# aous72/OpenJPH

Hardware: AMD Instinct MI355X
Metric: Msamples/s encode+decode, 8K 12-bit 4:4:4; achieved HBM GB/s vs roofline (higher is better)
Workload: dtype f32; 1 GPU; c3_8k_444_12b_irv97; width=7680, height=4320, components=3, bit_depth=12, wavelet=9/7 irreversible, decomps=5, hip_streams=1, sample_container_bits=16, roundtrip_max_abs_err=8

## Files before the change

openjph_amd/csrc/kernels_ht_dec.hip:

```cpp
#include <hip/hip_runtime.h>
#include <algorithm>
#include <cstdlib>
#include <stdint.h>
#include <type_traits>
#include "../../include/ojphgpu.h"
#include "ht_quant.h"
#include "ht_tables.h"
#include "ht_uvlc.h"

namespace ojphgpu {
__device__ uint16_t g_dec_vlc[2][1024];
__device__ uint32_t g_dec_vlc32[2][1024];
__device__ uint16_t g_dec_uvlc0[320];
}

namespace {

using ojphgpu::dequantise;

constexpr int WAVES = 4;
constexpr uint32_t RING_WORDS = 256;
constexpr uint32_t RING_MASK = RING_WORDS - 1;
constexpr uint32_t RING_ALLOC = RING_WORDS + 2;
constexpr uint32_t ROW_BITS_MAX = 64 * 2 * 32;
// ... 174 lines not shown
  __device__ __forceinline__ void prefetch() { pre = w[idx < last ? idx : last]; }
  __device__ __forceinline__ void settle() {}
};

typedef __attribute__((address_space(3))) uint32_t lds_u32;
constexpr uint32_t LDS_WAIT_SPINS = 1u << 23;
constexpr uint32_t EV_WORDS = 44;
constexpr uint32_t EV_RING = 8;
__device__ __forceinline__ uint32_t ev_words_of(uint32_t QW, uint32_t QH)
{
  const uint32_t w = (QW * QH + ((QW + 1u) >> 1) + 31u) / 32u + 2u;
  return w < EV_WORDS ? w : EV_WORDS;
}

constexpr uint32_t EV_AHEAD = 4;
__device__ __forceinline__ void mel_run(uint64_t& win, uint32_t& n, uint32_t& k, uint64_t& ev, uint32_t& nev)
{
  const uint32_t e = mel_exp(k);
  const uint32_t top = (uint32_t)(win >> 32);
  const bool zr = (top >> 31) != 0u;
  const uint32_t run = (top >> (31u - e)) & ((1u << e) - 1u);
  const uint32_t adv = zr ? 1u : e + 1u;
  ev |= zr ? 0ull : 1ull << (nev + run);
  nev += zr ? 1u << e : run + 1u;
  k = zr ? (k < 12u ? k + 1u : 12u) : (k > 0u ? k - 1u : 0u);
  win <<= adv; n -= adv;
}

__device__ __forceinline__ void mel_producer(const uint32_t* __restrict__ w, uint32_t nwords, uint32_t out_words,
                                             lds_u32* s_ev, volatile lds_u32* s_prog, const volatile lds_u32* s_cons,
                                             const volatile lds_u32* s_done, uint32_t lane)
{
  const uint32_t last = nwords - 1u;
  uint64_t win = ((uint64_t)w[0] << 32) | (uint64_t)w[last < 1u ? last : 1u];
  uint32_t n = 64, idx = 2, k = 0, nev = 0, wr = 0;
  uint32_t pre = w[last < 2u ? last : 2u];
  uint64_t ev = 0;
  while (wr < out_words && s_done[lane] == 0u) {
    const bool go = wr < s_cons[lane] + EV_AHEAD;
    if (go) {
      if (n <= 32u) { win |= (uint64_t)pre << (32u - n); n += 32u; ++idx; pre = w[idx < last ? idx : last]; }
      while (nev <= 31u && n >= 6u) mel_run(win, n, k, ev, nev);
      if (nev >= 32u) {
        s_ev[(wr & (EV_RING - 1u)) * 64u + lane] = (uint32_t)ev; ev >>= 32; nev -= 32u; ++wr;
        __builtin_amdgcn_fence(__ATOMIC_RELEASE, "workgroup", "local");
        s_prog[lane] = wr;
      }
    }
    if (__ballot(go) == 0ull) __builtin_amdgcn_s_sleep(16);
  }
}

struct EvRd {
  const lds_u32* ev; volatile lds_u32* prog; volatile lds_u32* cons; uint32_t idx, last, lo, hi, pre, bp, avail, lane; bool stuck;
  __device__ __forceinline__ uint32_t fetch(uint32_t want) {
    if (want >= avail && !stuck) {
      uint32_t spins = 0;
      do { __builtin_amdgcn_s_sleep(2); avail = prog[lane]; } while (want >= avail && ++spins < LDS_WAIT_SPINS);
      __builtin_amdgcn_fence(__ATOMIC_ACQUIRE, "workgroup", "local");
      stuck = stuck || want >= avail;
    }
    return ev[(want & (EV_RING - 1u)) * 64u + lane];
  }
  __device__ __forceinline__ void init(const lds_u32* e, volatile lds_u32* p, volatile lds_u32* c, uint32_t nwords, uint32_t l) {
    ev = e; prog = p; cons = c; last = nwords - 1u; lane = l; avail = 0; stuck = false;
    lo = fetch(0); hi = fetch(last < 1u ? last : 1u); pre = fetch(last < 2u ? last : 2u);
    idx = 2; bp = 0;
  }
  __device__ __forceinline__ uint32_t peek() const { return __builtin_amdgcn_alignbit(hi, lo, bp); }
  __device__ __forceinline__ void advance(uint32_t k) {
    bp += k;
    const bool cross = bp >= 32u;
    lo = cross ? hi : lo; hi = cross ? pre : hi;
    bp = cross ? bp - 32u : bp; idx += cross ? 1u : 0u;
  }
  __device__ __forceinline__ void prefetch() { cons[lane] = idx; pre = fetch(idx < last ? idx : last); }
};

struct __attribute__((aligned(4))) U2 { uint32_t x, y; };
__device__ __forceinline__ void store_pair(uint32_t* p, uint32_t a, uint32_t b)
{
  U2 v; v.x = a; v.y = b;
  *reinterpret_cast<U2*>(p) = v;
}

constexpr uint32_t REC_STRIDE = 128;

#define PIN_WINDOW(r) asm volatile("" : "+v"((r).lo), "+v"((r).hi))

#ifndef S2_ROWS_N
#define S2_ROWS_N 8
#endif
constexpr uint32_t S2_ROWS = S2_ROWS_N, S2_MAX_PER_WAVE = 8;
struct SliceSched {
  uint32_t tail, b1, b2, max_qh, n;
  uint32_t h1, h2;
  __host__ __device__ explicit SliceSched(uint32_t mq) {
    max_qh = mq ? mq : 1u;
    tail = ((max_qh - 1u) / S2_ROWS) * S2_ROWS;
#ifndef S2_TAIL
#define S2_TAIL 2
#endif
    b1 = (S2_TAIL >= 1 && max_qh > tail + 4u) ? max_qh - 4u : tail;
    b2 = (S2_TAIL >= 2 && max_qh > b1 + 2u) ? max_qh - 2u : b1;
#ifndef S2_HEAD
#define S2_HEAD 0
#endif
    const bool head = S2_HEAD != 0 && tail >= S2_ROWS && S2_ROWS == 8u;
    h1 = !head ? 0u : S2_HEAD == 1 ? 4u : 2u;
    h2 = !head ? 0u : S2_HEAD == 2 ? 4u : 0u;
    n = tail / S2_ROWS + 1u + (b1 > tail ? 1u : 0u) + (b2 > b1 ? 1u : 0u) + (h1 ? 1u : 0u) + (h2 ? 1u : 0u);
  }
  __host__ __device__ void bounds(uint32_t sl, uint32_t& lo, uint32_t& hi) const {
    const uint32_t extra = (h1 ? 1u : 0u) + (h2 ? 1u : 0u);
    if (sl <= extra) {
      const uint32_t first_end = tail >= S2_ROWS ? S2_ROWS : 0u;
      if (extra && first_end) {
        const uint32_t c0 = 0u, c1 = h1, c2 = h2 ? h2 : first_end, c3 = first_end;
        if (sl == 0u) { lo = c0; hi = c1; return; }
        if (sl == 1u) { lo = c1; hi = c2; return; }
        lo = c2; hi = c3; return;
      }
    }
    sl -= extra;
    const uint32_t full = tail / S2_ROWS;
    if (sl < full) { lo = sl * S2_ROWS; hi = lo + S2_ROWS; return; }
    uint32_t j = sl - full;
    lo = tail;
    if (b1 > tail) { if (j == 0u) { hi = b1; return; } --j; lo = b1; }
    if (b2 > b1) { if (j == 0u) { hi = b2; return; } --j; lo = b2; }
// ... 11 lines not shown
  u32x4 q[4];
#pragma unroll
  for (uint32_t j = 0; j < 4; ++j) {
    q[j].x = s_rec[(4 * j + 0) * 64 + lane]; q[j].y = s_rec[(4 * j + 1) * 64 + lane];
    q[j].z = s_rec[(4 * j + 2) * 64 + lane]; q[j].w = s_rec[(4 * j + 3) * 64 + lane];
  }
  asm volatile("global_store_dwordx4 %0, %1, off sc1\n\tglobal_store_dwordx4 %0, %2, off offset:1024 sc1\n\t"
               "global_store_dwordx4 %0, %3, off offset:2048 sc1\n\tglobal_store_dwordx4 %0, %4, off offset:3072 sc1"
               :: "v"(dst), "v"(q[0]), "v"(q[1]), "v"(q[2]), "v"(q[3]) : "memory");
}
#ifdef FUSED_TIMELINE
__device__ uint32_t g_tl_pub[1024 * 8];
__device__ uint32_t* g_tl_flags;
#endif
__device__ __forceinline__ void publish_rows(uint32_t* flag, uint32_t epoch, uint32_t rows, uint32_t lane)
{
#ifdef FUSED_TIMELINE
  const uint32_t tl_a = (uint32_t)__builtin_amdgcn_s_memrealtime();
#endif
  asm volatile("s_waitcnt vmcnt(0)" ::: "memory");
  if (lane == (uint32_t)__builtin_ctzll(__ballot(1))) {
    st_agent(flag, (epoch << 16) | rows);
#ifdef FUSED_TIMELINE
    const uint32_t k = rows == 0xFFFFu ? 7u : (rows & 7u) ? 8u : (rows >> 3) - 1u;
    if (k < 8u) { g_tl_pub[((flag - g_tl_flags) & 1023u) * 8u + k] = (uint32_t)__builtin_amdgcn_s_memrealtime(); if (k < 4u) g_tl_pub[((flag - g_tl_flags) & 1023u) * 8u + 4u + k] = tl_a; }
#endif
  }
}

template <class VlcRd>
__device__ __forceinline__ void uvlc_extension(VlcRd& vlc, uint32_t& used, uint32_t& u0, uint32_t& u1, uint32_t b0, uint32_t b1)
{
  const bool c0 = u0 - b0 > 32u, c1 = u1 - b1 > 32u;
  if (__ballot(c0 | c1) == 0ull) return;
  vlc.settle(); vlc.advance(used); vlc.prefetch(); vlc.settle(); used = 0;
  uint32_t v = vlc.peek();
  if (c0) { u0 += (v & 0xFu) << 2; v >>= 4; used += 4u; }
  if (c1) { u1 += (v & 0xFu) << 2; used += 4u; }
}

template <int NARROW, bool FUSED = false, bool W64 = false, class VlcRd, class TblT>
__device__ __forceinline__ void step1_rows(VlcRd& vlc, EvRd& mel, uint32_t* __restrict__ rec, uint32_t QW, uint32_t QH,
                                           const TblT* s_vlc, const uint16_t* s_uvlc0, uint32_t* flag = nullptr, uint32_t epoch = 0,
                                           lds_u32* s_rec = nullptr, SliceSched sched = SliceSched(S2_ROWS))
{
  static_assert(!FUSED || NARROW == 1, "the fused launch's records are for blocks of at most 64 columns");
  typedef typename std::conditional<NARROW == 2, unsigned __int128, uint64_t>::type Mask;
  auto row16 = [&](uint32_t qy_) { return rec + (size_t)qy_ * (64u * REC16_ROW_WORDS); };
  Mask sig_prev = 0;
  const uint32_t PW = (QW + 1) >> 1;

  {
    uint32_t tleft = 0; Mask sig_cur = 0;
    for (uint32_t qx = 0; qx < QW; qx += 2) {
      uint32_t v = vlc.peek(), used = 0;
      const uint32_t evq = mel.peek(); uint32_t ecnt = 0;
      uint32_t c_q = ((tleft & 0x10u) << 3) | ((tleft & 0xE0u) << 2);
      uint32_t t0 = s_vlc[c_q + (v & 0x7Fu)];
      if (c_q == 0) { if (((evq >> ecnt) & 1u) == 0) t0 = 0; ecnt++; }
      v >>= (t0 & 7u); used += t0 & 7u;
      uint32_t t1 = 0;
      if (qx + 1 < QW) {
        c_q = ((t0 & 0x10u) << 3) | ((t0 & 0xE0u) << 2);
        t1 = s_vlc[c_q + (v & 0x7Fu)];
        if (c_q == 0) { if (((evq >> ecnt) & 1u) == 0) t1 = 0; ecnt++; }
        v >>= (t1 & 7u); used += t1 & 7u;
      }
      tleft = t1;
      if (NARROW) {
        const uint32_t nib = FUSED ? (((t0 >> 9) & 3u) | ((t1 >> 7) & 0xCu))
                                   : (((t0 >> 5) & 1u) | ((t0 >> 6) & 2u) | ((t1 >> 3) & 4u) | ((t1 >> 4) & 8u));
        sig_cur |= (Mask)nib << (2u * qx);
      }
      uint32_t mode = ((t0 & 0x8u) << 3) | ((t1 & 0x8u) << 4);
      if (mode == 0xC0u) { if ((evq >> ecnt) & 1u) mode += 0x40u; ecnt++; }
      uint32_t entry = s_uvlc0[mode + (v & 0x3Fu)];
      v >>= (entry & 7u); used += entry & 7u; entry >>= 3;
      uint32_t len = entry & 0xFu;
      const uint32_t tmp = v & ((1u << len) - 1u);
      used += len; entry >>= 4;
      len = entry & 7u; entry >>= 3;
      uint32_t u0 = 1u + (entry & 7u) + (tmp & ~(0xFFu << len));
      uint32_t u1 = 1u + (entry >> 3) + (tmp >> len);
      if (W64) { const uint32_t bias = mode == 0x100u ? 3u : 1u; uvlc_extension(vlc, used, u0, u1, bias, bias); }
      vlc.settle(); vlc.advance(used); PIN_WINDOW(vlc); vlc.prefetch(); mel.advance(ecnt); mel.prefetch();
      if (FUSED) s_rec[(qx >> 1) * 64u + vlc.lane] = (t0 >> 16) | (u0 << 9) | (t1 & 0xFFFF0000u) | (u1 << 25);
      else store_pair(rec + (size_t)(qx >> 1) * REC_STRIDE, (uint32_t)t0 | (u0 << 16), (uint32_t)t1 | (u1 << 16));
    }
    if (FUSED) flush_row16(s_rec, vlc.lane, row16(0));
    sig_prev = sig_cur;
  }
  const TblT* tbl = s_vlc + 1024;
  for (uint32_t qy = 1; qy < QH; ++qy) {
    uint32_t* row = rec + (size_t)qy * PW * REC_STRIDE;
    const uint32_t* above = row - (size_t)PW * REC_STRIDE;
    auto above_rec = [&](uint32_t q) { return above[(size_t)(q >> 1) * REC_STRIDE + (q & 1u)]; };
    uint32_t tleft = 0; Mask sig_cur = 0;
    const Mask sig_or = sig_prev | (sig_prev >> 1);
    uint32_t carry = ((uint32_t)sig_prev & 1u) << 7;
    for (uint32_t qx = 0; qx < QW; qx += 2) {
      uint32_t v = vlc.peek(), used = 0;
      const uint32_t evq = mel.peek(); uint32_t ecnt = 0;
      uint32_t k0, k1;
      if (NARROW) {
        const uint32_t w = (uint32_t)(sig_or >> (2u * qx));
        k0 = carry | ((w & 2u) << 8);
        k1 = (w & 0xAu) << 6;
        carry = (w & 8u) << 4;
      } else {
        const uint32_t up0 = above_rec(qx);
        const uint32_t upl = qx ? above_rec(qx - 1) : 0u;
        const uint32_t up1 = qx + 1 < QW ? above_rec(qx + 1) : 0u;
        const uint32_t up2 = qx + 2 < QW ? above_rec(qx + 2) : 0u;
        const uint32_t sg = ((upl >> 7) & 1u) | (((up0 >> 5) & 1u) << 1) | (((up0 >> 7) & 1u) << 2) | (((up1 >> 5) & 1u) << 3) |
                            (((up1 >> 7) & 1u) << 4) | (((up2 >> 5) & 1u) << 5);
        k0 = (((sg | (sg >> 1)) & 1u) << 7) | ((((sg >> 2) | (sg >> 3)) & 1u) << 9);
        k1 = ((((sg >> 2) | (sg >> 3)) & 1u) << 7) | ((((sg >> 4) | (sg >> 5)) & 1u) << 9);
      }
      const uint32_t c_q0 = FUSED ? ((tleft & 0x100u) | k0) : (((tleft & 0x40u) << 2) | ((tleft & 0x80u) << 1) | k0);
      uint32_t t0 = tbl[c_q0 + (v & 0x7Fu)];
      const bool z0 = c_q0 == 0;
      t0 = (z0 & ((evq & 1u) == 0)) ? 0u : t0;
      ecnt = z0 ? 1u : 0u;
      v >>= (t0 & 7u); used += t0 & 7u;
      const bool ex1 = qx + 1 < QW;
      const uint32_t c_q1 = FUSED ? ((t0 & 0x100u) | k1) : (((t0 & 0x40u) << 2) | ((t0 & 0x80u) << 1) | k1);
      uint32_t t1 = tbl[c_q1 + (v & 0x7Fu)];
      const bool z1 = ex1 & (c_q1 == 0);
      t1 = ((!ex1) | (z1 & (((evq >> ecnt) & 1u) == 0))) ? 0u : t1;
      ecnt += z1 ? 1u : 0u;
      v >>= (t1 & 7u); used += t1 & 7u;
      tleft = t1;
      if (NARROW) {
        const uint32_t nib = FUSED ? (((t0 >> 9) & 3u) | ((t1 >> 7) & 0xCu))
                                   : (((t0 >> 5) & 1u) | ((t0 >> 6) & 2u) | ((t1 >> 3) & 4u) | ((t1 >> 4) & 8u));
        sig_cur |= (Mask)nib << (2u * qx);
      }
      uint32_t u0, u1;
      used += ojphgpu::uvlc_pair_other_rows(v, t0 & 0x8u, t1 & 0x8u, u0, u1);
      if (W64) uvlc_extension(vlc, used, u0, u1, 0u, 0u);
      vlc.settle(); vlc.advance(used); PIN_WINDOW(vlc); vlc.prefetch(); mel.advance(ecnt); mel.prefetch();
      if (FUSED) s_rec[(qx >> 1) * 64u + vlc.lane] = (t0 >> 16) | (u0 << 9) | (t1 & 0xFFFF0000u) | (u1 << 25);
      else store_pair(row + (size_t)(qx >> 1) * REC_STRIDE, (uint32_t)t0 | (u0 << 16), (uint32_t)t1 | (u1 << 16));
    }
    if (FUSED) flush_row16(s_rec, vlc.lane, row16(qy));
    sig_prev = sig_cur;
    if (FUSED && sched.publishes_after(qy + 1u)) publish_rows(flag, epoch, qy + 1u, vlc.lane);
  }
}

constexpr uint32_t VR_WORDS = 16, VR_LOW = 6, EV_LOW = 2;
#ifndef MEL_RUNS_PER_PASS
#define MEL_RUNS_PER_PASS 16
#endif

struct RingRd {
  const lds_u32* ring; volatile lds_u32* prog; volatile lds_u32* cons; uint32_t idx, lo, hi, pre, bp, av, pidx, lane; bool stuck;
  __device__ __forceinline__ uint32_t fetch(uint32_t want) {
    if (stuck) return 0u;
    uint32_t avail = prog[lane], spins = 0;
    while (want >= avail && ++spins < LDS_WAIT_SPINS) { __builtin_amdgcn_s_sleep(2); avail = prog[lane]; }

    __builtin_amdgcn_fence(__ATOMIC_ACQUIRE, "workgroup", "local");
    stuck = stuck || want >= avail;
    return ring[(want & (VR_WORDS - 1u)) * 64u + lane];
  }
  __device__ __forceinline__ void init(const lds_u32* r, volatile lds_u32* p, volatile lds_u32* c, uint32_t l) {
    ring = r; prog = p; cons = c; lane = l; stuck = false;
    lo = fetch(0); hi = fetch(1); pre = fetch(2);
    idx = 2; bp = 0; pidx = 0; av = 1;
  }
  __device__ __forceinline__ uint32_t peek() const { return __builtin_amdgcn_alignbit(hi, lo, bp); }
  __device__ __forceinline__ void advance(uint32_t k) {
    bp += k;
    const bool cross = bp >= 32u;
    lo = cross ? hi : lo; hi = cross ? pre : hi;
    bp = cross ? bp - 32u : bp; idx += cross ? 1u : 0u;
  }
  __device__ __forceinline__ void prefetch() { cons[lane] = idx; pidx = idx; av = prog[lane]; pre = ring[(idx & (VR_WORDS - 1u)) * 64u + lane]; }
  __device__ __forceinline__ void settle() {
    if (pidx >= av) {
      pre = fetch(pidx); av = pidx + 1u;
    }
  }
};

struct __attribute__((aligned(4))) B16 { uint32_t d[4]; };
__device__ __forceinline__ B16 load_b16_unaligned(const uint8_t* p) { B16 v; __builtin_memcpy(&v, p, 16); return v; }

template <int ROLE>
__device__ __forceinline__ void raw_partner(const uint8_t* __restrict__ cb, uint32_t lcup, uint32_t scup, uint32_t room_below,
                                            const B16& v0, const B16& v1, uint32_t ev_words,
                                            lds_u32* s_ev, volatile lds_u32* s_eprog, const volatile lds_u32* s_econs,
                                            lds_u32* s_vr, volatile lds_u32* s_vprog, const volatile lds_u32* s_vcons,
                                            const volatile lds_u32* s_done, uint32_t lane)
{
  const uint32_t vreal = scup - 2u, vcount = vreal + 1u;
  const uint32_t d0 = cb[lcup - 2];
  uint64_t vacc = d0 >> 4;
  uint32_t vnb = 4u - ((((d0 >> 4) & 7u) == 7u) ? 1u : 0u);
  uint32_t vk = 0, vwr = 0, vp1 = d0 | 0xFu;
  bool vp1_short = false;
  auto vload = [&](uint32_t k) -> B16 {
    B16 z; z.d[0] = z.d[1] = z.d[2] = z.d[3] = 0u;
    if (k >= vcount) return z;
    const int off = (int)lcup - 18 - (int)k;
    if (off >= -(int)room_below) return load_b16_unaligned(cb + off);
    for (int j = 0; j < 16; ++j) {
      const int o = off + 15 - j;
      if (o >= 0) z.d[3 - (j >> 2)] |= (uint32_t)cb[o] << (24 - 8 * (j & 3));
    }
    return z;
  };
  B16 vcur = v0, vnext = v1;
  const uint32_t mcount = scup - 1u, moff = lcup - scup;
  auto mload = [&](uint32_t k) -> B16 {
    if (k < mcount) return load_b16_unaligned(cb + moff + k);
    B16 z; z.d[0] = z.d[1] = z.d[2] = z.d[3] = 0xFFFFFFFFu; return z;
  };
  uint64_t win = 0;
  uint32_t n = 0, mk = 0, mprev = 0, k = 0, nev = 0, ewr = 0;
// ... 68 lines not shown
template <int CH>
__global__ __launch_bounds__(192 * CH) void ht_dec_step1_raw_kernel(
    const ojphgpu_cb_desc* __restrict__ blocks, uint32_t n, const uint8_t* __restrict__ data,
    uint32_t* __restrict__ quads, uint8_t* __restrict__ block_status)
{
  __shared__ uint16_t s_vlc[2048];
  __shared__ uint16_t s_uvlc0[320];
  __shared__ uint32_t s_ev_all[CH][EV_RING * 64];
  __shared__ uint32_t s_vr_all[CH][VR_WORDS * 64];
  __shared__ uint32_t s_ctl_all[CH][5][64];
  for (int i = threadIdx.x; i < 2048; i += blockDim.x) s_vlc[i] = (&ojphgpu::g_dec_vlc[0][0])[i];
  for (int i = threadIdx.x; i < 320; i += blockDim.x) s_uvlc0[i] = ojphgpu::g_dec_uvlc0[i];
  for (int i = threadIdx.x; i < CH * 5 * 64; i += blockDim.x) (&s_ctl_all[0][0][0])[i] = 0;
  __syncthreads();

  const uint32_t lane = threadIdx.x & 63u;
  const uint32_t wv = (uint32_t)__builtin_amdgcn_readfirstlane((int)(threadIdx.x >> 6));
  const bool chain = wv < (uint32_t)CH;
  const uint32_t set = wv % (uint32_t)CH;
  lds_u32* s_ev = (lds_u32*)s_ev_all[set];
  lds_u32* s_vr = (lds_u32*)s_vr_all[set];
  volatile lds_u32* s_eprog = (volatile lds_u32*)s_ctl_all[set][0];
  volatile lds_u32* s_econs = (volatile lds_u32*)s_ctl_all[set][1];
  volatile lds_u32* s_vprog = (volatile lds_u32*)s_ctl_all[set][2];
  volatile lds_u32* s_vcons = (volatile lds_u32*)s_ctl_all[set][3];
  volatile lds_u32* s_done = (volatile lds_u32*)s_ctl_all[set][4];
  if (chain) __builtin_amdgcn_s_setprio(3);
  const uint32_t bi = (blockIdx.x * (uint32_t)CH + set) * 64u + lane;
  if (bi >= n) return;
  const ojphgpu_cb_desc d = blocks[bi];
  if (d.reversible & 4u) return;
  if (d.w == 0 || d.h == 0 || d.len1 == 0 || d.num_passes == 0) { if (chain) block_status[bi] = 0; return; }
  const uint8_t* cb = data + d.data_off;
  const uint32_t room = d.data_off > 0xFFFFu ? 0xFFFFu : (uint32_t)d.data_off;
  B16 v0, v1;
  v0.d[0] = v0.d[1] = v0.d[2] = v0.d[3] = 0u; v1 = v0;
  if (!chain && wv < 2u * (uint32_t)CH) {
    const int o0 = (int)d.len1 - 18, o1 = o0 - 16;
    if (o0 >= -(int)room) v0 = load_b16_unaligned(cb + o0);
    else for (int j = 0; j < 16; ++j) { const int o = o0 + 15 - j; if (o >= 0) v0.d[3 - (j >> 2)] |= (uint32_t)cb[o] << (24 - 8 * (j & 3)); }
    if (o1 >= -(int)room) v1 = load_b16_unaligned(cb + o1);
    else for (int j = 0; j < 16; ++j) { const int o = o1 + 15 - j; if (o >= 0) v1.d[3 - (j >> 2)] |= (uint32_t)cb[o] << (24 - 8 * (j & 3)); }
  }
  const uint32_t scup = check_block(d, cb);
  if (scup == 0) { if (chain) block_status[bi] = 1; return; }
  const uint32_t QW = ((uint32_t)d.w + 1) >> 1, QH = ((uint32_t)d.h + 1) >> 1;
  const uint32_t evw = ev_words_of(QW, QH);
  if (!chain) {
    if (wv < 2u * (uint32_t)CH) raw_partner<1>(cb, d.len1, scup, room, v0, v1, evw, s_ev, s_eprog, s_econs, s_vr, s_vprog, s_vcons, s_done, lane);
    else raw_partner<2>(cb, d.len1, scup, room, v0, v1, evw, s_ev, s_eprog, s_econs, s_vr, s_vprog, s_vcons, s_done, lane);
    return;
  }
  uint32_t* rec = quads + d.scratch_cap;
  RingRd vlc; vlc.init(s_vr, s_vprog, s_vcons, lane);
  EvRd mel; mel.init(s_ev, s_eprog, s_econs, evw, lane);
  if (__all(QW <= 32)) step1_rows<1>(vlc, mel, rec, QW, QH, s_vlc, s_uvlc0);
  else if (__all(QW <= 64)) step1_rows<2>(vlc, mel, rec, QW, QH, s_vlc, s_uvlc0);
  else step1_rows<0>(vlc, mel, rec, QW, QH, s_vlc, s_uvlc0);
  s_done[lane] = 1u;
  block_status[bi] = (mel.stuck || vlc.stuck) ? 1 : 0;
}

template <int CH, bool W64 = false>
__global__ __launch_bounds__(128 * CH) void ht_dec_step1_kernel(
    const ojphgpu_cb_desc* __restrict__ blocks, uint32_t n, const uint8_t* __restrict__ data,
    const uint32_t* __restrict__ aux, uint32_t* __restrict__ quads, uint8_t* __restrict__ block_status)
{
  __shared__ uint16_t s_vlc[2048];
  __shared__ uint16_t s_uvlc0[320];
  __shared__ uint32_t s_ev_all[CH][EV_RING * 64];
  __shared__ uint32_t s_prog_all[CH][64];
  __shared__ uint32_t s_done_all[CH][64];
  __shared__ uint32_t s_cons_all[CH][64];
  for (int i = threadIdx.x; i < 2048; i += blockDim.x) s_vlc[i] = (&ojphgpu::g_dec_vlc[0][0])[i];
  for (int i = threadIdx.x; i < 320; i += blockDim.x) s_uvlc0[i] = ojphgpu::g_dec_uvlc0[i];
  if (threadIdx.x < 64 * CH) { (&s_prog_all[0][0])[threadIdx.x] = 0; (&s_done_all[0][0])[threadIdx.x] = 0; (&s_cons_all[0][0])[threadIdx.x] = 0; }
  __syncthreads();

  const uint32_t lane = threadIdx.x & 63u;
  const uint32_t wv = (uint32_t)__builtin_amdgcn_readfirstlane((int)(threadIdx.x >> 6));
  const bool chain = wv < (uint32_t)CH;
  const uint32_t set = chain ? wv : wv - (uint32_t)CH;
  uint32_t* s_ev = s_ev_all[set];
  uint32_t* s_prog = s_prog_all[set];
  volatile lds_u32* s_done = (volatile lds_u32*)s_done_all[set];
  volatile lds_u32* s_cons = (volatile lds_u32*)s_cons_all[set];
  if (chain) __builtin_amdgcn_s_setprio(3);
  const uint32_t bi = (blockIdx.x * (uint32_t)CH + set) * 64u + lane;
  if (bi >= n) return;
  const ojphgpu_cb_desc d = blocks[bi];
  if (((d.reversible & 4u) != 0) != W64) return;
  if (d.w == 0 || d.h == 0 || d.len1 == 0 || d.num_passes == 0) { if (chain) block_status[bi] = 0; return; }
  const uint8_t* cb = data + d.data_off;
  const uint32_t scup = check_block(d, cb);
  if (scup == 0) { if (chain) block_status[bi] = 1; return; }
  const uint32_t QW = ((uint32_t)d.w + 1) >> 1, QH = ((uint32_t)d.h + 1) >> 1;
  const uint32_t evw = ev_words_of(QW, QH);
  if (!chain) {
    mel_producer(aux + d.reserved + vlc_words(scup), mel_words(scup), evw, (lds_u32*)s_ev, (volatile lds_u32*)s_prog, s_cons, s_done, lane);
    return;
  }
  uint32_t* rec = quads + d.scratch_cap;

  FlatRd vlc; vlc.init(aux + d.reserved, vlc_words(scup));
  EvRd mel; mel.init((const lds_u32*)s_ev, (volatile lds_u32*)s_prog, s_cons, evw, lane);

  if (__all(QW <= 32)) step1_rows<1, false, W64>(vlc, mel, rec, QW, QH, s_vlc, s_uvlc0);
  else if (__all(QW <= 64)) step1_rows<2, false, W64>(vlc, mel, rec, QW, QH, s_vlc, s_uvlc0);
  else step1_rows<0, false, W64>(vlc, mel, rec, QW, QH, s_vlc, s_uvlc0);
  s_done[lane] = 1u;
  block_status[bi] = mel.stuck ? 1 : 0;
}


#ifndef S2_ABL
#define S2_ABL 0
#endif
__device__ __forceinline__ bool needs_refinement(const ojphgpu_cb_desc& d)
{
  return d.num_passes > 1 && d.num_passes <= 3 && d.len2 > 0 && (d.missing_msbs < 29 || (d.reversible & 4u));
}

constexpr uint32_t S2_STATE_WORDS = 24;

#ifdef FUSED_TIMELINE
__device__ uint32_t g_tl[8192 * 12];
__device__ __forceinline__ uint32_t tl_now() { return (uint32_t)__builtin_amdgcn_s_memrealtime(); }
#endif
constexpr uint32_t TICKET_STRIDE = 32;
constexpr uint32_t TICKET_CU_WORDS = 8 * 256;
constexpr uint32_t TICKET_WORDS = TICKET_CU_WORDS + 2 * TICKET_STRIDE;

__device__ __forceinline__ uint32_t rec16_base(const ojphgpu_cb_desc& d, uint32_t bi)
{
  const uint32_t l = bi & 63u;
  return d.scratch_cap - 2u * l + l * 4u;
}

__device__ __forceinline__ void load_slice_records(const uint32_t* __restrict__ quads, const ojphgpu_cb_desc& d, uint32_t bi,
                                                   uint32_t qy_begin, uint32_t qy_end, int lane, uint32_t* ents)
{
  const uint32_t QH = ((uint32_t)d.h + 1u) >> 1;
  const uint16_t* r16 = reinterpret_cast<const uint16_t*>(quads + rec16_base(d, bi) + (size_t)qy_begin * (64u * REC16_ROW_WORDS) + ((uint32_t)lane >> 4) * 256u)
                        + (((uint32_t)lane >> 1) & 7u);
  constexpr uint32_t row_step = 2u * 64u * REC16_ROW_WORDS;
  const uint32_t last = (qy_end < QH ? qy_end : QH) - qy_begin - 1u;
#pragma unroll
  for (uint32_t i = 0; i < S2_ROWS; ++i)
    ents[i] = (uint32_t)__hip_atomic_load(r16 + (i < last ? i : last) * row_step, __ATOMIC_RELAXED, __HIP_MEMORY_SCOPE_AGENT);
}

template <int TX, int WD, bool SLICED, bool KEEP = false>
__device__ __forceinline__ void step2_block(const ojphgpu_cb_desc& d, uint32_t bi, const uint8_t* __restrict__ data,
                                            const uint32_t* __restrict__ quads, uint32_t* __restrict__ coef,
                                            uint8_t* __restrict__ block_status, uint32_t* ring, uint8_t* s_exp_w,
                                            int lane, uint32_t qy_begin, uint32_t qy_end, uint32_t* state, bool prepare = false)
{
  const uint32_t W = d.w, H = d.h, pitch = d.pitch;
  if (W == 0 || H == 0) return;
  uint32_t* dst = coef + d.coef_off;
  const bool rev = TX == 1 ? true : TX == 2 ? false : (d.reversible & 1u) != 0;
  const uint32_t K = d.K_max;
  const bool raw_out = TX ? false : needs_refinement(d);

// ... 52 lines not shown
  if (wide) for (uint32_t i = lane; i < 2 * EXP_BYTES / 4; i += 64) reinterpret_cast<uint32_t*>(s_exp_w)[i] = 0;
  wave_sync();

  uint32_t dst_bits = 0, src_pos = 0, mpos = 0;
  uint32_t hs[5] = { 0, 0, 0, 0, 0 }, hd[5] = { 0, 0, 0, 0, 0 };
  auto unstuff_chunk = [&]() {
    if (SLICED && !KEEP) {
#pragma unroll
      for (int i = 4; i > 0; --i) { hs[i] = hs[i - 1]; hd[i] = hd[i - 1]; }
      hs[0] = src_pos; hd[0] = dst_bits;
    }
    const uint32_t wb = (dst_bits + 31u) >> 5;
    {
      const uint32_t z0 = (wb + (uint32_t)lane) & RING_MASK;
      ring[z0] = 0;
      if (z0 < 2u) ring[z0 + RING_WORDS] = 0;
      if (lane < 2) { const uint32_t z1 = (wb + 64u + (uint32_t)lane) & RING_MASK; ring[z1] = 0; if (z1 < 2u) ring[z1 + RING_WORDS] = 0; }
    }
    wave_sync();
    const uint32_t i0 = src_pos + 4u * (uint32_t)lane;
    uint32_t val = 0, nb = 0;
    const uint32_t word = i0 < ms_len ? load_u32_unaligned(cb + i0) : 0u;
    uint32_t pw = from_prev(word);
    if (lane == 0) pw = (i0 && i0 < ms_len) ? load_u32_unaligned(cb + i0 - 4) : 0u;
    asm volatile("" :: "v"(word), "v"(pw));
    if (i0 < ms_len) {
      const uint32_t cnt = min(4u, ms_len - i0);
      const uint32_t valid = cnt == 4u ? 0xFFFFFFFFu : (1u << (8u * cnt)) - 1u;
      const uint32_t P = (word << 8) | (pw >> 24), P2 = (word << 16) | (pw >> 16);
      auto is_ff = [](uint32_t x) { return ((x & 0x7F7F7F7Fu) + 0x01010101u) & x & 0x80808080u; };
      const uint32_t S = is_ff(P) & valid;
      const uint32_t stray = (is_ff(P2) >> 7) & (P >> 7) & 0x01010101u;
      uint32_t x = ((word | stray) & valid) & ~S;
      x = (S & 0x00800000u) ? (x & 0x007FFFFFu) | ((x >> 1) & 0xFF800000u) : x;
      x = (S & 0x00008000u) ? (x & 0x00007FFFu) | ((x >> 1) & 0xFFFF8000u) : x;
      x = (S & 0x00000080u) ? (x & 0x0000007Fu) | ((x >> 1) & 0xFFFFFF80u) : x;
      val = x;
      nb = 8u * cnt - (uint32_t)__popc(S);
    }
    const uint32_t incl = wave_incl_scan(nb);
    const uint32_t pos = dst_bits + incl - nb;
    if (nb) {
      const uint32_t w = pos >> 5, sh = pos & 31;
      const uint32_t wa = w & RING_MASK, wb2 = (w + 1) & RING_MASK;
      atomicOr(&ring[wa], val << sh);
      if (wa < 2u) atomicOr(&ring[wa + RING_WORDS], val << sh);
      if (sh + nb > 32) { atomicOr(&ring[wb2], val >> (32 - sh)); if (wb2 < 2u) atomicOr(&ring[wb2 + RING_WORDS], val >> (32 - sh)); }
    }
    dst_bits += rdlane(incl, 63);
    src_pos += 256;
    wave_sync();
  };

  const uint32_t mmsbp2 = missing_msbs + 2;
  const uint32_t shift = 31 - K;
  const float delta = d.delta;
  const uint32_t half = (uint32_t)lane & 1u;
  bool bad = false;
  uint32_t e_prev = 0;
  if (KEEP && prepare) {
    while (src_pos < ms_len && dst_bits < ROW_BITS_MAX + 64u) unstuff_chunk();
    if (lane < 16) state[lane] = 0u;
    if (lane == 0) { state[16] = 0u; state[17] = src_pos; state[18] = dst_bits; state[19] = 0u; state[20] = ms_len; }
    wave_sync();
    return;
  }
  if (SLICED && (KEEP || qy_begin > 0)) {
    if (!KEEP && rdfirst(state[19]) != 0u) return;
    e_prev = (state[(uint32_t)lane >> 2] >> (8u * ((uint32_t)lane & 3u))) & 0xFFu;
    mpos = rdfirst(state[16]); src_pos = rdfirst(state[17]); dst_bits = rdfirst(state[18]);
    hs[0] = src_pos; hd[0] = dst_bits;
  }
  uint32_t ent_next = 0;
  if (!SLICED) {
    ent_next = (uint32_t)lane < W && qy_begin < qy_last ? rec_at(qy_begin, (uint32_t)lane >> 1) : 0u;
    asm volatile("" : "+v"(ent_next));
  }
  for (uint32_t qy = qy_begin; qy < qy_last && !bad; ++qy) {
    const uint8_t* vexp = s_exp_w + (qy & 1) * EXP_BYTES;
    uint8_t* vnew = s_exp_w + ((qy & 1) ^ 1) * EXP_BYTES;
    for (uint32_t c0 = 0; c0 < (WD == 1 ? 1u : W); c0 += 64) {
      while (!(S2_ABL & 16) && src_pos < ms_len && (int32_t)(dst_bits - mpos) < (int32_t)(ROW_BITS_MAX + 64u)) unstuff_chunk();
      const bool exhausted = src_pos >= ms_len;
      const uint32_t col = c0 + (uint32_t)lane;
      const bool act = col < W;
      const uint32_t qx = col >> 1;
      const uint32_t ent = SLICED ? ents[0] : ent_next;
      if (SLICED) {
#pragma unroll
        for (uint32_t i = 0; i + 1 < (SLICED ? S2_ROWS : 1u); ++i) ents[i] = ents[i + 1];
      } else {
        uint32_t nc0 = c0 + 64, nqy = qy;
        if (nc0 >= W) { nc0 = 0; nqy = qy + 1; }
        const uint32_t ncol = nc0 + (uint32_t)lane;
        ent_next = (nqy < qy_last && ncol < W) ? rec_at(nqy, ncol >> 1) : 0u;
      }
      const uint32_t inf = act ? (ent & 0xFFFFu) : 0u;
      uint32_t U_q = SLICED ? inf >> 9 : ent >> 16;
      if (qy > 0) {
        uint32_t gamma = SLICED ? inf & 0x100u : inf & 0xF0u;
        if (!SLICED) gamma &= gamma - 0x10u;
        uint32_t em;
        if (S2_ABL & 8) em = e_prev;
        else if (!wide) {
          const uint32_t e_nx = from_next(e_prev), e_pv = from_prev(e_prev);
          const uint32_t hm = max(e_prev, half ? e_nx : e_pv);
          em = max(hm, from_pair(hm));
        } else {
          const uint32_t b = 2 * qx;
          em = act ? max(max((uint32_t)vexp[b], (uint32_t)vexp[b + 1]), max((uint32_t)vexp[b + 2], (uint32_t)vexp[b + 3])) : 0u;
        }
        U_q += gamma ? max(em, 1u) : 1u;
      }
      if (__ballot(U_q > mmsbp2) != 0ull) { bad = true; break; }
      const uint32_t sel = SLICED ? inf >> (4u * half) : inf >> (2u * half);
      const uint32_t st0 = sel & 3u, st1 = (sel >> 2) & 3u;
      const bool sg0 = SLICED ? st0 != 0u : (sel & 0x10u) != 0u, sg1 = SLICED ? st1 != 0u : (sel & 0x20u) != 0u;
      const uint32_t ek0 = SLICED ? st0 >> 1 : (sel >> 12) & 1u, ek1 = SLICED ? st1 >> 1 : (sel >> 13) & 1u;
      const uint32_t eb0 = SLICED ? st0 & (st0 >> 1) : (sel >> 8) & 1u, eb1 = SLICED ? st1 & (st1 >> 1) : (sel >> 9) & 1u;
      const uint32_t m0 = sg0 ? U_q - ek0 : 0u;
      const uint32_t m1 = sg1 ? U_q - ek1 : 0u;
      const uint32_t tot = m0 + m1;
      const uint32_t incl = (S2_ABL & 2) ? tot * ((uint32_t)lane + 1u) : wave_incl_scan(tot);
      const uint32_t at = mpos + incl - tot;
      mpos += (S2_ABL & 2) ? 64u : rdlane(incl, 63);
      const uint32_t wi = at >> 5, sh = at & 31;
      const uint32_t* rw = ring + (wi & RING_MASK);
      const uint32_t w0 = (S2_ABL & 4) ? at : rw[0], w1 = (S2_ABL & 4) ? at * 3u : rw[1], w2 = (S2_ABL & 4) ? at * 5u : rw[2];
      uint64_t win = (uint64_t)__funnelshift_r(w0, w1, sh) | ((uint64_t)__funnelshift_r(w1, w2, sh) << 32);
      if (exhausted) {
        if (at >= dst_bits) win = ~0ull;
        else if (at + 64 > dst_bits) win |= ~0ull << (dst_bits - at);
      }
      uint32_t out0, out1, v1;
      {
        const uint32_t ms_val = (uint32_t)win;
        uint32_t v_n = ms_val & ((1u << m0) - 1u);
        v_n |= eb0 << m0;
        v_n |= 1u;
        const uint32_t val = ((ms_val << 31) | ((v_n + 2u) << (p - 1))) & (sg0 ? 0xFFFFFFFFu : 0u);
        out0 = raw_out ? val : dequantise(val, rev, shift, delta);
      }
      {
        const uint32_t ms_val = __builtin_amdgcn_alignbit((uint32_t)(win >> 32), (uint32_t)win, m0);
        uint32_t v_n = ms_val & ((1u << m1) - 1u);
        v_n |= eb1 << m1;
        v_n |= 1u;
        const uint32_t keep = sg1 ? 0xFFFFFFFFu : 0u;
        const uint32_t val = ((ms_val << 31) | ((v_n + 2u) << (p - 1))) & keep;
        v1 = v_n & keep;
        out1 = raw_out ? val : dequantise(val, rev, shift, delta);
      }
      const uint32_t e_new = v1 ? 31u - (uint32_t)__clz((int)v1) : 0u;
      if (!wide) e_prev = e_new;
      else if (act) vnew[col + 1] = (uint8_t)e_new;
      if (!SLICED) asm volatile("" : "+v"(ent_next));
      if (act && (!(S2_ABL & 1) || (out0 ^ out1) == 0x9E3779B9u)) {
        const uint32_t y = 2 * qy;
        char* rowp = reinterpret_cast<char*>(dst + (size_t)y * pitch);
        char* rowp1 = rowp + (size_t)pitch * 4u;
        uint32_t coff = col * 4u;
        asm volatile("" : "+v"(coff));
        *reinterpret_cast<uint32_t*>(rowp + coff) = out0;
        if (y + 1 < H) { asm volatile("" : "+v"(coff)); *reinterpret_cast<uint32_t*>(rowp1 + coff) = out1; }
      }
    }
    if (wide) wave_sync();
  }
  if (bad) { zero_block(); if (lane == 0) block_status[bi] = 1; }
  if (SLICED && qy_last < QH) {
    if (bad) { if (lane == 0) state[19] = 1u; wave_sync(); return; }
    uint32_t rs = hs[4], rd = hd[4];
#pragma unroll
    for (int i = 3; i >= 0; --i) if (hd[i] <= mpos) { rs = hs[i]; rd = hd[i]; }
    if (KEEP) { rs = src_pos; rd = dst_bits; }
    const uint32_t e4 = e_prev | (from_next(e_prev) << 8);
    const uint32_t e8 = e4 | ((uint32_t)__builtin_amdgcn_update_dpp(0, (int)e4, 0x102, 0xF, 0xF, false) << 16);
    if (((uint32_t)lane & 3u) == 0) state[(uint32_t)lane >> 2] = e8;
    if (lane == 0) { state[16] = mpos; state[17] = rs; state[18] = rd; state[19] = 0u; }
    wave_sync();
  }
}

template <int TX, int WD>
__global__ __launch_bounds__(64 * WAVES) void ht_dec_step2_kernel(
    const ojphgpu_cb_desc* __restrict__ blocks, uint32_t n, const uint8_t* __restrict__ data,
    const uint32_t* __restrict__ quads, uint32_t* __restrict__ coef, uint8_t* __restrict__ block_status)
{
  __shared__ uint32_t s_ring[WAVES][RING_ALLOC];
  __shared__ uint8_t s_exp[WAVES][2][EXP_BYTES];
  const int lane = threadIdx.x & 63;
  const int wave = __builtin_amdgcn_readfirstlane((int)(threadIdx.x >> 6));
  const uint32_t q8 = gridDim.x >> 3, r8 = gridDim.x & 7u, xcd = blockIdx.x & 7u;
  const uint32_t wg = xcd * q8 + (xcd < r8 ? xcd : r8) + (blockIdx.x >> 3);
  const uint32_t bi = wg * WAVES + wave;
  if (bi >= n) return;
  const ojphgpu_cb_desc d = blocks[bi];
  if (d.reversible & 4u) return;
  step2_block<TX, WD, false>(d, bi, data, quads, coef, block_status, s_ring[wave], &s_exp[wave][0][0], lane, 0u, 0xFFFFFFFFu, nullptr);
}



template <int LPB>
__device__ __forceinline__ uint32_t seg_incl_scan(uint32_t v)
{
  int x = (int)v;
  x += __builtin_amdgcn_update_dpp(0, x, 0x111, 0xF, 0xF, false);
  x += __builtin_amdgcn_update_dpp(0, x, 0x112, 0xF, 0xF, false);
  x += __builtin_amdgcn_update_dpp(0, x, 0x114, 0xF, 0xF, false);
  x += __builtin_amdgcn_update_dpp(0, x, 0x118, 0xF, 0xF, false);
  if (LPB == 32) x += __builtin_amdgcn_update_dpp(0, x, 0x142, 0xA, 0xF, false);
  return (uint32_t)x;
}
template <int LPB>
__device__ __forceinline__ uint32_t seg_last(uint32_t v, uint32_t seg)
{
  if (LPB == 32) { const uint32_t a = rdlane(v, 31), b = rdlane(v, 63); return seg ? b : a; }
  const uint32_t a = rdlane(v, 15), b = rdlane(v, 31), c = rdlane(v, 47), d = rdlane(v, 63);
  return seg & 2u ? (seg & 1u ? d : c) : (seg & 1u ? b : a);
// ... 372 lines not shown
  for (int i = threadIdx.x; i < 320; i += blockDim.x) s_uvlc0[i] = ojphgpu::g_dec_uvlc0[i];
  for (int i = threadIdx.x; i < CH * 5 * 64; i += blockDim.x) s_mem[CTL_OFF + i] = 0;
  __syncthreads();
  if (wv >= 3u * (uint32_t)CH) return;
  const bool chain = wv < (uint32_t)CH;
  const uint32_t set = wv % (uint32_t)CH;
  lds_u32* s_ev = (lds_u32*)(s_mem + EV_OFF + set * EV_RING * 64);
  lds_u32* s_vr = (lds_u32*)(s_mem + VR_OFF + set * VR_WORDS * 64);
  uint32_t* const ctl = s_mem + CTL_OFF + set * 5 * 64;
  volatile lds_u32* s_eprog = (volatile lds_u32*)(ctl);
  volatile lds_u32* s_econs = (volatile lds_u32*)(ctl + 64);
  volatile lds_u32* s_vprog = (volatile lds_u32*)(ctl + 128);
  volatile lds_u32* s_vcons = (volatile lds_u32*)(ctl + 192);
  volatile lds_u32* s_done = (volatile lds_u32*)(ctl + 256);
#ifndef PARTNER_PRIO
#define PARTNER_PRIO 2
#endif
  if (chain) __builtin_amdgcn_s_setprio(3);
  else if (PARTNER_PRIO) __builtin_amdgcn_s_setprio(PARTNER_PRIO);
  const uint32_t cw = wgid * (uint32_t)CH + set;
  const uint32_t bi = cw * 64u + lane;
  uint32_t* flag = fstate + cw;
  bool alive = bi < n;
  ojphgpu_cb_desc d = blocks[alive ? bi : 0];
  if (alive && (d.w == 0 || d.h == 0 || d.len1 == 0 || d.num_passes == 0)) {
    if (chain) __hip_atomic_store(block_status + bi, (uint8_t)0, __ATOMIC_RELAXED, __HIP_MEMORY_SCOPE_AGENT);
    alive = false;
  }
  const uint8_t* cb = data + d.data_off;
  const uint32_t room = d.data_off > 0xFFFFu ? 0xFFFFu : (uint32_t)d.data_off;
  B16 v0, v1;
  v0.d[0] = v0.d[1] = v0.d[2] = v0.d[3] = 0u; v1 = v0;
  if (alive && !chain && wv < 2u * (uint32_t)CH) {
    const int o0 = (int)d.len1 - 18, o1 = o0 - 16;
    if (o0 >= -(int)room) v0 = load_b16_unaligned(cb + o0);
    else for (int jj = 0; jj < 16; ++jj) { const int o = o0 + 15 - jj; if (o >= 0) v0.d[3 - (jj >> 2)] |= (uint32_t)cb[o] << (24 - 8 * (jj & 3)); }
    if (o1 >= -(int)room) v1 = load_b16_unaligned(cb + o1);
    else for (int jj = 0; jj < 16; ++jj) { const int o = o1 + 15 - jj; if (o >= 0) v1.d[3 - (jj >> 2)] |= (uint32_t)cb[o] << (24 - 8 * (jj & 3)); }
  }
  uint32_t scup = 0;
  if (alive) {
    scup = check_block(d, cb);
    if (scup == 0) { if (chain) __hip_atomic_store(block_status + bi, (uint8_t)1, __ATOMIC_RELAXED, __HIP_MEMORY_SCOPE_AGENT); alive = false; }
  }
  if (alive) {
    const uint32_t QW = ((uint32_t)d.w + 1) >> 1, QH = ((uint32_t)d.h + 1) >> 1;
    const uint32_t evw = ev_words_of(QW, QH);
    if (!chain) {
      if (wv < 2u * (uint32_t)CH) raw_partner<1>(cb, d.len1, scup, room, v0, v1, evw, s_ev, s_eprog, s_econs, s_vr, s_vprog, s_vcons, s_done, lane);
      else raw_partner<2>(cb, d.len1, scup, room, v0, v1, evw, s_ev, s_eprog, s_econs, s_vr, s_vprog, s_vcons, s_done, lane);
    } else {
      __hip_atomic_store(block_status + bi, (uint8_t)0, __ATOMIC_RELAXED, __HIP_MEMORY_SCOPE_AGENT);
      uint32_t* rec = quads + rec16_base(d, bi);
      RingRd vlc; vlc.init(s_vr, s_vprog, s_vcons, lane);
      EvRd mel; mel.init(s_ev, s_eprog, s_econs, evw, lane);
      step1_rows<1, true>(vlc, mel, rec, QW, QH, s_vlc, s_uvlc0, flag, epoch, (lds_u32*)(s_mem + REC_OFF + set * REC16_ROW_WORDS * 64), sched);
      s_done[lane] = 1u;
      if (mel.stuck || vlc.stuck) ask_for_repeat(retry, host_retry, epoch);
    }
  }
  if (chain) publish_rows(flag, epoch, 0xFFFFu, lane);
#ifdef FUSED_TIMELINE
  if (lane == 0) {
    uint32_t* tl = g_tl + (size_t)((wgid * (uint32_t)WGW + wv) & 8191u) * 12u;
    tl[0] = chain ? 1u : 3u; tl[1] = tl_where; tl[2] = tl_t0; tl[3] = tl_now();
  }
#endif
}


constexpr int RWAVES = 2;
constexpr uint32_t SIG_ENTRIES = 1040;
constexpr uint32_t PREV_ENTRIES = 264;

template <typename S>
struct RefineLds {
  S smp[4096];
  uint16_t sigma[SIG_ENTRIES];
  uint16_t prev_row[PREV_ENTRIES];
  uint8_t  bytes[2048];
};

struct FwdBits {
  const uint8_t* d; int i, n_bytes; uint64_t win; uint32_t n, unstuff;
  __device__ __forceinline__ void init(const uint8_t* p, int len) { d = p; i = 0; n_bytes = len; win = 0; n = 0; unstuff = 0; }
  __device__ __forceinline__ uint32_t bit() {
    if (n == 0) {
      const uint32_t b = i < n_bytes ? d[i] : 0u; ++i;
      win |= (uint64_t)b;
      n = 8u - unstuff; unstuff = (b == 0xFFu);
    }
    const uint32_t r = (uint32_t)win & 1u; win >>= 1; --n;
    return r;
  }
};

struct BwdBits {
  const uint8_t* d; int i; uint64_t win; uint32_t n, unstuff;
  __device__ __forceinline__ void init(const uint8_t* p, int len) { d = p; i = len - 1; win = 0; n = 0; unstuff = 1; }
  __device__ __forceinline__ uint32_t bit() {
    if (n == 0) {
      const uint32_t b = i >= 0 ? d[i] : 0u; --i;
      win |= (uint64_t)b;
      n = 8u - ((unstuff && (b & 0x7Fu) == 0x7Fu) ? 1u : 0u); unstuff = b > 0x8Fu;
    }
    const uint32_t r = (uint32_t)win & 1u; win >>= 1; --n;
    return r;
  }
};

__device__ __forceinline__ void sigma_from_records(const uint32_t* __restrict__ rec, uint32_t QW, uint32_t QH, uint16_t* sigma,
// ... 665 lines not shown
```

Before: 104,400 Msamples/s.

## Batch MEL event-bit consumption per quad group and share give-up flag in LDS

The step-1 decoder now peeks one 32-bit MEL event word per group of quads and advances or prefetches the MEL reader once per group, instead of once per quad pair. This cuts the LDS ring polling and fences in the inner loop. The per-reader 'stuck' booleans are replaced by a shared per-lane give-up flag in LDS (reusing s_done), which costs an LDS read on each fetch. Step 2 gets small cleanups: the row pointer is strength-reduced across rows, the p-1 shift is hoisted, and the neighbour-max exponent is simplified. Together these remove VGPR and ALU work. Risks: a group may consume more than 32 event bits, narrow blocks treat the whole row as one group, and reusing s_done as the give-up flag could interact with the partner wave's termination check.

```diff
diff --git a/openjph_amd/csrc/kernels_ht_dec.hip b/openjph_amd/csrc/kernels_ht_dec.hip
--- a/openjph_amd/csrc/kernels_ht_dec.hip
+++ b/openjph_amd/csrc/kernels_ht_dec.hip
@@ -250,18 +250,20 @@
 }
 
 struct EvRd {
-  const lds_u32* ev; volatile lds_u32* prog; volatile lds_u32* cons; uint32_t idx, last, lo, hi, pre, bp, avail, lane; bool stuck;
+  const lds_u32* ev; volatile lds_u32* prog; volatile lds_u32* cons; volatile lds_u32* gave_up; uint32_t idx, last, lo, hi, pre, bp, avail, lane;
   __device__ __forceinline__ uint32_t fetch(uint32_t want) {
-    if (want >= avail && !stuck) {
-      uint32_t spins = 0;
-      do { __builtin_amdgcn_s_sleep(2); avail = prog[lane]; } while (want >= avail && ++spins < LDS_WAIT_SPINS);
-      __builtin_amdgcn_fence(__ATOMIC_ACQUIRE, "workgroup", "local");
-      stuck = stuck || want >= avail;
+    if (want >= avail) {
+      if (gave_up[lane] == 0u) {
+        uint32_t spins = 0;
+        do { __builtin_amdgcn_s_sleep(2); avail = prog[lane]; } while (want >= avail && ++spins < LDS_WAIT_SPINS);
+        __builtin_amdgcn_fence(__ATOMIC_ACQUIRE, "workgroup", "local");
+        if (want >= avail) gave_up[lane] = 2u;
+      }
     }
     return ev[(want & (EV_RING - 1u)) * 64u + lane];
   }
-  __device__ __forceinline__ void init(const lds_u32* e, volatile lds_u32* p, volatile lds_u32* c, uint32_t nwords, uint32_t l) {
-    ev = e; prog = p; cons = c; last = nwords - 1u; lane = l; avail = 0; stuck = false;
+  __device__ __forceinline__ void init(const lds_u32* e, volatile lds_u32* p, volatile lds_u32* c, volatile lds_u32* g, uint32_t nwords, uint32_t l) {
+    ev = e; prog = p; cons = c; gave_up = g; last = nwords - 1u; lane = l; avail = 0;
     lo = fetch(0); hi = fetch(last < 1u ? last : 1u); pre = fetch(last < 2u ? last : 2u);
     idx = 2; bp = 0;
   }
@@ -273,7 +275,9 @@
     bp = cross ? bp - 32u : bp; idx += cross ? 1u : 0u;
   }
   __device__ __forceinline__ void prefetch() { cons[lane] = idx; pre = fetch(idx < last ? idx : last); }
+  __device__ __forceinline__ bool stuck() const { return gave_up[lane] == 2u; }
 };
+constexpr uint32_t EV_GROUP0 = 16, EV_GROUP = 32;
 
 struct __attribute__((aligned(4))) U2 { uint32_t x, y; };
 __device__ __forceinline__ void store_pair(uint32_t* p, uint32_t a, uint32_t b)
@@ -391,9 +395,12 @@
 
   {
     uint32_t tleft = 0; Mask sig_cur = 0;
-    for (uint32_t qx = 0; qx < QW; qx += 2) {
+    for (uint32_t qg = 0; qg < QW; qg += EV_GROUP0) {
+    const uint32_t qe = qg + EV_GROUP0 < QW ? qg + EV_GROUP0 : QW;
+    uint32_t evq = mel.peek(), etot = 0;
+    for (uint32_t qx = qg; qx < qe; qx += 2) {
       uint32_t v = vlc.peek(), used = 0;
-      const uint32_t evq = mel.peek(); uint32_t ecnt = 0;
+      uint32_t ecnt = 0;
       uint32_t c_q = ((tleft & 0x10u) << 3) | ((tleft & 0xE0u) << 2);
       uint32_t t0 = s_vlc[c_q + (v & 0x7Fu)];
       if (c_q == 0) { if (((evq >> ecnt) & 1u) == 0) t0 = 0; ecnt++; }
@@ -422,9 +429,12 @@
       uint32_t u0 = 1u + (entry & 7u) + (tmp & ~(0xFFu << len));
       uint32_t u1 = 1u + (entry >> 3) + (tmp >> len);
       if (W64) { const uint32_t bias = mode == 0x100u ? 3u : 1u; uvlc_extension(vlc, used, u0, u1, bias, bias); }
-      vlc.settle(); vlc.advance(used); PIN_WINDOW(vlc); vlc.prefetch(); mel.advance(ecnt); mel.prefetch();
+      vlc.settle(); vlc.advance(used); PIN_WINDOW(vlc); vlc.prefetch();
+      evq >>= ecnt; etot += ecnt;
       if (FUSED) s_rec[(qx >> 1) * 64u + vlc.lane] = (t0 >> 16) | (u0 << 9) | (t1 & 0xFFFF0000u) | (u1 << 25);
       else store_pair(rec + (size_t)(qx >> 1) * REC_STRIDE, (uint32_t)t0 | (u0 << 16), (uint32_t)t1 | (u1 << 16));
+    }
+    mel.advance(etot); mel.prefetch();
     }
     if (FUSED) flush_row16(s_rec, vlc.lane, row16(0));
     sig_prev = sig_cur;
@@ -437,9 +447,12 @@
     uint32_t tleft = 0; Mask sig_cur = 0;
     const Mask sig_or = sig_prev | (sig_prev >> 1);
     uint32_t carry = ((uint32_t)sig_prev & 1u) << 7;
-    for (uint32_t qx = 0; qx < QW; qx += 2) {
+    for (uint32_t qg = 0; qg < (NARROW == 1 ? 1u : QW); qg += EV_GROUP) {
+    const uint32_t qe = (NARROW != 1 && qg + EV_GROUP < QW) ? qg + EV_GROUP : QW;
+    uint32_t evq = mel.peek(), etot = 0;
+    for (uint32_t qx = qg; qx < qe; qx += 2) {
       uint32_t v = vlc.peek(), used = 0;
-      const uint32_t evq = mel.peek(); uint32_t ecnt = 0;
+      uint32_t ecnt = 0;
       uint32_t k0, k1;
       if (NARROW) {
         const uint32_t w = (uint32_t)(sig_or >> (2u * qx));
@@ -478,9 +491,12 @@
       uint32_t u0, u1;
       used += ojphgpu::uvlc_pair_other_rows(v, t0 & 0x8u, t1 & 0x8u, u0, u1);
       if (W64) uvlc_extension(vlc, used, u0, u1, 0u, 0u);
-      vlc.settle(); vlc.advance(used); PIN_WINDOW(vlc); vlc.prefetch(); mel.advance(ecnt); mel.prefetch();
+      vlc.settle(); vlc.advance(used); PIN_WINDOW(vlc); vlc.prefetch();
+      evq >>= ecnt; etot += ecnt;
       if (FUSED) s_rec[(qx >> 1) * 64u + vlc.lane] = (t0 >> 16) | (u0 << 9) | (t1 & 0xFFFF0000u) | (u1 << 25);
       else store_pair(row + (size_t)(qx >> 1) * REC_STRIDE, (uint32_t)t0 | (u0 << 16), (uint32_t)t1 | (u1 << 16));
+    }
+    mel.advance(etot); mel.prefetch();
     }
     if (FUSED) flush_row16(s_rec, vlc.lane, row16(qy));
     sig_prev = sig_cur;
@@ -494,18 +510,18 @@
 #endif
 
 struct RingRd {
-  const lds_u32* ring; volatile lds_u32* prog; volatile lds_u32* cons; uint32_t idx, lo, hi, pre, bp, av, pidx, lane; bool stuck;
+  const lds_u32* ring; volatile lds_u32* prog; volatile lds_u32* cons; volatile lds_u32* gave_up; uint32_t idx, lo, hi, pre, bp, av, pidx, lane;
   __device__ __forceinline__ uint32_t fetch(uint32_t want) {
-    if (stuck) return 0u;
+    if (gave_up[lane] != 0u) return 0u;
     uint32_t avail = prog[lane], spins = 0;
     while (want >= avail && ++spins < LDS_WAIT_SPINS) { __builtin_amdgcn_s_sleep(2); avail = prog[lane]; }
 
     __builtin_amdgcn_fence(__ATOMIC_ACQUIRE, "workgroup", "local");
-    stuck = stuck || want >= avail;
+    if (want >= avail) gave_up[lane] = 2u;
     return ring[(want & (VR_WORDS - 1u)) * 64u + lane];
   }
-  __device__ __forceinline__ void init(const lds_u32* r, volatile lds_u32* p, volatile lds_u32* c, uint32_t l) {
-    ring = r; prog = p; cons = c; lane = l; stuck = false;
+  __device__ __forceinline__ void init(const lds_u32* r, volatile lds_u32* p, volatile lds_u32* c, volatile lds_u32* g, uint32_t l) {
+    ring = r; prog = p; cons = c; gave_up = g; lane = l;
     lo = fetch(0); hi = fetch(1); pre = fetch(2);
     idx = 2; bp = 0; pidx = 0; av = 1;
   }
@@ -680,13 +696,14 @@
     return;
   }
   uint32_t* rec = quads + d.scratch_cap;
-  RingRd vlc; vlc.init(s_vr, s_vprog, s_vcons, lane);
-  EvRd mel; mel.init(s_ev, s_eprog, s_econs, evw, lane);
+  RingRd vlc; vlc.init(s_vr, s_vprog, s_vcons, s_done, lane);
+  EvRd mel; mel.init(s_ev, s_eprog, s_econs, s_done, evw, lane);
   if (__all(QW <= 32)) step1_rows<1>(vlc, mel, rec, QW, QH, s_vlc, s_uvlc0);
   else if (__all(QW <= 64)) step1_rows<2>(vlc, mel, rec, QW, QH, s_vlc, s_uvlc0);
   else step1_rows<0>(vlc, mel, rec, QW, QH, s_vlc, s_uvlc0);
+  const bool gave_up = mel.stuck();
   s_done[lane] = 1u;
-  block_status[bi] = (mel.stuck || vlc.stuck) ? 1 : 0;
+  block_status[bi] = gave_up ? 1 : 0;
 }
 
 template <int CH, bool W64 = false>
@@ -731,13 +748,14 @@
   uint32_t* rec = quads + d.scratch_cap;
 
   FlatRd vlc; vlc.init(aux + d.reserved, vlc_words(scup));
-  EvRd mel; mel.init((const lds_u32*)s_ev, (volatile lds_u32*)s_prog, s_cons, evw, lane);
+  EvRd mel; mel.init((const lds_u32*)s_ev, (volatile lds_u32*)s_prog, s_cons, s_done, evw, lane);
 
   if (__all(QW <= 32)) step1_rows<1, false, W64>(vlc, mel, rec, QW, QH, s_vlc, s_uvlc0);
   else if (__all(QW <= 64)) step1_rows<2, false, W64>(vlc, mel, rec, QW, QH, s_vlc, s_uvlc0);
   else step1_rows<0, false, W64>(vlc, mel, rec, QW, QH, s_vlc, s_uvlc0);
+  const bool gave_up = mel.stuck();
   s_done[lane] = 1u;
-  block_status[bi] = mel.stuck ? 1 : 0;
+  block_status[bi] = gave_up ? 1 : 0;
 }
 
 
@@ -896,7 +914,8 @@
     wave_sync();
   };
 
-  const uint32_t mmsbp2 = missing_msbs + 2;
+  uint32_t mmsbp2 = missing_msbs + 2, pm1 = p - 1;
+  if (SLICED) asm volatile("" : "+v"(mmsbp2), "+v"(pm1));
   const uint32_t shift = 31 - K;
   const float delta = d.delta;
   const uint32_t half = (uint32_t)lane & 1u;
@@ -920,6 +939,7 @@
     ent_next = (uint32_t)lane < W && qy_begin < qy_last ? rec_at(qy_begin, (uint32_t)lane >> 1) : 0u;
     asm volatile("" : "+v"(ent_next));
   }
+  char* rowp = reinterpret_cast<char*>(dst + (size_t)(2u * qy_begin) * pitch);
   for (uint32_t qy = qy_begin; qy < qy_last && !bad; ++qy) {
     const uint8_t* vexp = s_exp_w + (qy & 1) * EXP_BYTES;
     uint8_t* vnew = s_exp_w + ((qy & 1) ^ 1) * EXP_BYTES;
@@ -947,8 +967,7 @@
         uint32_t em;
         if (S2_ABL & 8) em = e_prev;
         else if (!wide) {
-          const uint32_t e_nx = from_next(e_prev), e_pv = from_prev(e_prev);
-          const uint32_t hm = max(e_prev, half ? e_nx : e_pv);
+          const uint32_t hm = max(from_prev(e_prev), from_next(e_prev));
           em = max(hm, from_pair(hm));
         } else {
           const uint32_t b = 2 * qx;
@@ -982,7 +1001,7 @@
         uint32_t v_n = ms_val & ((1u << m0) - 1u);
         v_n |= eb0 << m0;
         v_n |= 1u;
-        const uint32_t val = ((ms_val << 31) | ((v_n + 2u) << (p - 1))) & (sg0 ? 0xFFFFFFFFu : 0u);
+        const uint32_t val = ((ms_val << 31) | ((v_n + 2u) << pm1)) & (sg0 ? 0xFFFFFFFFu : 0u);
         out0 = raw_out ? val : dequantise(val, rev, shift, delta);
       }
       {
@@ -991,7 +1010,7 @@
         v_n |= eb1 << m1;
         v_n |= 1u;
         const uint32_t keep = sg1 ? 0xFFFFFFFFu : 0u;
-        const uint32_t val = ((ms_val << 31) | ((v_n + 2u) << (p - 1))) & keep;
+        const uint32_t val = ((ms_val << 31) | ((v_n + 2u) << pm1)) & keep;
         v1 = v_n & keep;
         out1 = raw_out ? val : dequantise(val, rev, shift, delta);
       }
@@ -1001,7 +1020,6 @@
       if (!SLICED) asm volatile("" : "+v"(ent_next));
       if (act && (!(S2_ABL & 1) || (out0 ^ out1) == 0x9E3779B9u)) {
         const uint32_t y = 2 * qy;
-        char* rowp = reinterpret_cast<char*>(dst + (size_t)y * pitch);
         char* rowp1 = rowp + (size_t)pitch * 4u;
         uint32_t coff = col * 4u;
         asm volatile("" : "+v"(coff));
@@ -1010,6 +1028,7 @@
       }
     }
     if (wide) wave_sync();
+    rowp += (size_t)pitch * 8u;
   }
   if (bad) { zero_block(); if (lane == 0) block_status[bi] = 1; }
   if (SLICED && qy_last < QH) {
@@ -1488,11 +1507,12 @@
     } else {
       __hip_atomic_store(block_status + bi, (uint8_t)0, __ATOMIC_RELAXED, __HIP_MEMORY_SCOPE_AGENT);
       uint32_t* rec = quads + rec16_base(d, bi);
-      RingRd vlc; vlc.init(s_vr, s_vprog, s_vcons, lane);
-      EvRd mel; mel.init(s_ev, s_eprog, s_econs, evw, lane);
+      RingRd vlc; vlc.init(s_vr, s_vprog, s_vcons, s_done, lane);
+      EvRd mel; mel.init(s_ev, s_eprog, s_econs, s_done, evw, lane);
       step1_rows<1, true>(vlc, mel, rec, QW, QH, s_vlc, s_uvlc0, flag, epoch, (lds_u32*)(s_mem + REC_OFF + set * REC16_ROW_WORDS * 64), sched);
+      const bool gave_up = mel.stuck();
       s_done[lane] = 1u;
-      if (mel.stuck || vlc.stuck) ask_for_repeat(retry, host_retry, epoch);
+      if (gave_up) ask_for_repeat(retry, host_retry, epoch);
     }
   }
   if (chain) publish_rows(flag, epoch, 0xFFFFu, lane);
```

New measurement: 106,000 Msamples/s, median of 6. About the same (+1.5%).
